# ChengZhang-98/lqer

Hardware: AMD Instinct MI355X
Metric: W4A8+rank-r Linear GEMM TFLOPS-equiv (higher is better)
Workload: dtype bf16; 1 GPU; LqerLinear 4096x4096 rank32 W4A8-MXINT16 M=2048 (BASELINE configs[1]); rank=32, formats=x MXINT8/16, W MXINT4/16, A_out,B_out as x, y fp16, weights=one Linear

## Files before the change

### lqer_amd/csrc/act16_fused.hip

```cpp
#include "common.h"

namespace lqer {
namespace a16f {

constexpr int ROWS = 8, WAVES = 8, SLAB = 512, PITCH = 1040;

__host__ inline size_t lds_bytes(int rp) { return (size_t)WAVES * ROWS * PITCH + (size_t)WAVES * ROWS * rp * sizeof(float); }

typedef __attribute__((ext_vector_type(8))) __bf16 bf16v8;

#ifdef LQER_CLOCKPROBE
__device__ unsigned long long* g_a16_stamp_buf = nullptr;
#define A16_STAMP(i) asm volatile("s_memtime %0\n\ts_waitcnt lgkmcnt(0)" : "=s"(cp[i])::"memory")
#else
#define A16_STAMP(i)
#endif

template <int DT, int RT>
__global__ __launch_bounds__(512) void k_act16_fused(const void* __restrict__ x, int64_t M, int64_t K, int64_t ld, QP qx, bf16_t* __restrict__ xq,
                                                      int64_t Kp, const bf16_t* __restrict__ a_frag, QP qa, int L_aout, bf16_t* __restrict__ xaq) {
  constexpr int RP = 16 * RT;
  constexpr int HB = RT == 8 ? 2 : (RT == 4 ? 4 : 8);
  constexpr int NPART = 16 / HB;
  extern __shared__ __attribute__((aligned(16))) unsigned char smem[];
  const int lane = threadIdx.x & 63;
  const int wave = __builtin_amdgcn_readfirstlane(threadIdx.x >> 6);
  unsigned char* const wb = smem + (size_t)wave * ROWS * PITCH;
  float* const red = (float*)(smem + (size_t)WAVES * ROWS * PITCH);
  const int64_t m0 = (int64_t)blockIdx.x * ROWS;
  const int nslab = (int)((Kp + SLAB - 1) / SLAB);
  const int g = lane >> 4;
  const unsigned char* const tok = wb + (lane & 7) * PITCH + 16 * g;
  const u32x4* const fr = (const u32x4*)a_frag + lane;
  f32x4 acc[RT];
#pragma unroll
  for (int t = 0; t < RT; ++t) acc[t] = (f32x4){0.f, 0.f, 0.f, 0.f};
#ifdef LQER_CLOCKPROBE
  unsigned long long cp[8] = {0, 0, 0, 0, 0, 0, 0, 0};
  A16_STAMP(0);
#endif

  for (int s = wave; s < nslab; s += WAVES) {
    const int64_t k0 = (int64_t)s * SLAB + 8 * lane;
    const bool in_img = k0 < Kp, in_x = k0 < K;
    u32x4 raw[ROWS];
#pragma unroll
    for (int r = 0; r < ROWS; ++r)
      raw[r] = (in_x && m0 + r < M) ? *(const u32x4*)((const bf16_t*)x + (m0 + r) * ld + k0) : (u32x4){0, 0, 0, 0};
    const int st0 = s * (SLAB / 32), nst = (int)(Kp / 32);
    u32x4 fa[HB][RT], fb[HB][RT];
    auto load_part = [&](u32x4 (&f)[HB][RT], int part) {
#pragma unroll
      for (int i = 0; i < HB; ++i)
#pragma unroll
        for (int t = 0; t < RT; ++t) {
          const int st = st0 + part * HB + i;
          f[i][t] = fr[((int64_t)(st < nst ? st : 0) * RT + t) * 64];
        }
    };
    if (s == wave) A16_STAMP(1);
#pragma unroll
    for (int r = 0; r < ROWS; ++r) {
      if (r == 1 && s == wave) A16_STAMP(2);
      if (r == 2) {
        asm volatile("" ::: "memory");
        load_part(fa, 0);
        asm volatile("" ::: "memory");
      }
      if (r == 5) {
        asm volatile("" ::: "memory");
        load_part(fb, 1);
        asm volatile("" ::: "memory");
      }
      float v[8];
      const uint32_t wd[4] = {raw[r][0], raw[r][1], raw[r][2], raw[r][3]};
#pragma unroll
      for (int j = 0; j < 4; ++j) {
        if constexpr (DT == LQER_F16) {
          typedef __attribute__((ext_vector_type(2))) _Float16 h2;
          const h2 h = __builtin_bit_cast(h2, wd[j]);
          v[2 * j] = (float)h[0], v[2 * j + 1] = (float)h[1];
        } else {
          v[2 * j] = __uint_as_float(wd[j] << 16), v[2 * j + 1] = __uint_as_float(wd[j] & 0xffff0000u);
        }
      }
      float amax = 0.f;
#pragma unroll
      for (int i = 0; i < 8; ++i) amax = fmaxf(amax, fabsf(v[i]));
      amax = fmaxf(amax, __shfl_xor(amax, 1, 64));
      uint32_t w[4] = {0, 0, 0, 0};
      if (amax > 0.f) {
        const int e = block_exponent_u(amax, qx);
        if (mxint16_fast_ok(e, qx)) {
          mxint16_bf16_fast<DT != LQER_F16, 8>(v, e, qx, w);
        } else {
#pragma unroll
          for (int i = 0; i < 4; ++i) {
            const uint32_t lo = exact_bf16_bits(ldexpf(mxint_mantissa(v[2 * i], e, qx), e - qx.mbits));
            const uint32_t hi = exact_bf16_bits(ldexpf(mxint_mantissa(v[2 * i + 1], e, qx), e - qx.mbits));
            w[i] = lo | (hi << 16);
          }
        }
      }
      const u32x4 wv = {w[0], w[1], w[2], w[3]};
      if (in_img) *(u32x4*)(xq + (m0 + r) * Kp + k0) = wv;
      *(u32x4*)(wb + r * PITCH + 16 * lane) = wv;
    }
    if (s == wave) A16_STAMP(3);
    __builtin_amdgcn_fence(__ATOMIC_RELEASE, "wavefront");
    __builtin_amdgcn_wave_barrier();
    __builtin_amdgcn_fence(__ATOMIC_ACQUIRE, "wavefront");
    auto half = [&](const u32x4 (&f)[HB][RT], int t0) {
      u32x4 tk[HB];
#pragma unroll
      for (int i = 0; i < HB; ++i) tk[i] = *(const u32x4*)(tok + 64 * (t0 + i));
#pragma unroll
      for (int i = 0; i < HB; ++i)
#pragma unroll
        for (int t = 0; t < RT; ++t)
          acc[t] = __builtin_amdgcn_mfma_f32_16x16x32_bf16(__builtin_bit_cast(bf16v8, tk[i]), __builtin_bit_cast(bf16v8, f[i][t]), acc[t], 0, 0, 0);
    };
#pragma unroll
    for (int pp = 0; pp < NPART; pp += 2) {
      half(fa, pp * HB);
      if (pp + 2 < NPART) load_part(fa, pp + 2);
      half(fb, (pp + 1) * HB);
      if (pp + 3 < NPART) load_part(fb, pp + 3);
    }
    __builtin_amdgcn_fence(__ATOMIC_RELEASE, "wavefront");
    __builtin_amdgcn_wave_barrier();
#ifdef LQER_CLOCKPROBE
    if (s == wave) {
      asm volatile("" ::"v"(acc[0]));
      A16_STAMP(4);
    }
#endif
  }
  if (g < 2) {
#pragma unroll
    for (int t = 0; t < RT; ++t)
#pragma unroll
      for (int j = 0; j < 4; ++j) red[(wave * ROWS + 4 * g + j) * RP + 16 * t + (lane & 15)] = acc[t][j];
  }
  __syncthreads();
#ifdef LQER_CLOCKPROBE
  A16_STAMP(5);
  if (g_a16_stamp_buf && lane == 0) {
    unsigned long long* o = g_a16_stamp_buf + ((size_t)blockIdx.x * WAVES + wave) * 8;
    for (int i = 1; i < 6; ++i) o[i] = cp[i] - cp[0];
    unsigned long long rt;
    asm volatile("s_memrealtime %0\n\ts_waitcnt lgkmcnt(0)" : "=s"(rt)::"memory");
    o[0] = cp[0], o[6] = rt;
  }
#endif
  const int tid = threadIdx.x;
  const bool live = tid < ROWS * RP / 4;
  const int r = tid / (RP / 4), c4 = tid - r * (RP / 4);
  float4 sum = make_float4(0.f, 0.f, 0.f, 0.f);
  if (live) {
#pragma unroll
    for (int w = 0; w < WAVES; ++w) {
      const float4 v = *(const float4*)(red + (w * ROWS + r) * RP + 4 * c4);
      sum.x += v.x, sum.y += v.y, sum.z += v.z, sum.w += v.w;
    }
  }
  if (tid >= 64 * ((ROWS * RP / 4 + 63) / 64)) return;
  float bmax = fmaxf(fmaxf(fabsf(sum.x), fabsf(sum.y)), fmaxf(fabsf(sum.z), fabsf(sum.w)));
  const int G = L_aout / 4;
  for (int d = 1; d < G; d <<= 1) bmax = fmaxf(bmax, __shfl_xor(bmax, d, 64));
  if (!live || m0 + r >= M) return;
  const bool anyb = bmax > 0.f;
  const int eb = anyb ? block_exponent(bmax, qa) : 0;
  const float v[4] = {sum.x, sum.y, sum.z, sum.w};
  uint32_t w2[2];
#pragma unroll
  for (int i = 0; i < 2; ++i) {
    const float m0v = anyb ? mxint_mantissa(v[2 * i], eb, qa) : 0.f;
    const float m1v = anyb ? mxint_mantissa(v[2 * i + 1], eb, qa) : 0.f;
    w2[i] = exact_bf16_bits(ldexpf(m0v, eb - qa.mbits)) | (exact_bf16_bits(ldexpf(m1v, eb - qa.mbits)) << 16);
  }
  *(uint2*)(xaq + ((m0 + r) * RP + 4 * c4)) = make_uint2(w2[0], w2[1]);
}

__global__ __launch_bounds__(256) void k_a_b16(const bf16_t* __restrict__ limb0, int64_t Kp, int rp, bf16_t* __restrict__ out) {
  const int RT = rp / 16;
  const int64_t n_img = (int64_t)rp * Kp / 8, total = 2 * n_img;
  for (int64_t idx = (int64_t)blockIdx.x * 256 + threadIdx.x; idx < total; idx += (int64_t)gridDim.x * 256) {
    if (idx < n_img) {
      ((u32x4*)out)[idx] = ((const u32x4*)limb0)[idx];
    } else {
      const int64_t f = idx - n_img;
      const int lane = (int)(f & 63);
      const int64_t blk = f >> 6;
      const int t = (int)(blk % RT);
      const int64_t s = blk / RT;
      ((u32x4*)out)[idx] = *(const u32x4*)(limb0 + (int64_t)(16 * t + (lane & 15)) * Kp + 32 * s + 8 * (lane >> 4));
    }
  }
}

}

#ifdef LQER_CLOCKPROBE
extern "C" int lqer_debug_set_a16_stamp_buffer(void* p) { return (int)hipMemcpyToSymbol(HIP_SYMBOL(a16f::g_a16_stamp_buf), &p, sizeof(p)); }
#endif

size_t a_b16_image_bytes(int64_t K, int64_t r) { return (size_t)2 * lqer_padded_r(r) * lqer_padded_k(K) * sizeof(bf16_t); }

int a_b16_prepare_dispatch(const void* a_t_limbs, int64_t K, int64_t r, void* out, hipStream_t st) {
  const int64_t rp = lqer_padded_r(r), Kp = lqer_padded_k(K);
  if (rp % 16 != 0 || Kp % 32 != 0) {
    set_error("a_b16_prepare: padded rank %d / padded K %d", (int)rp, (int)Kp);
    return LQER_E_UNSUPPORTED;
  }
  const int64_t total = 2 * rp * Kp / 8;
  a16f::k_a_b16<<<(unsigned)((total + 255) / 256 < 4096 ? (total + 255) / 256 : 4096), 256, 0, st>>>((const bf16_t*)a_t_limbs, Kp, (int)rp, (bf16_t*)out);
  return check_launch("a_b16_prepare");
}

int act16_fused_dispatch(const void* x, int dtype, int64_t M, int64_t K, int64_t ldx, const QP& qx, bf16_t* xq, const void* a_b16, int64_t r,
                         const QP& qa, bf16_t* xaq, int tuning, hipStream_t st) {
  if (tuning & LQER_TUNE_ACT16_SPLIT) return LQER_E_UNSUPPORTED;
  const int64_t rp = lqer_padded_r(r), Kp = lqer_padded_k(K);
  if (dtype == LQER_F32 || !a_b16 || !xaq || !xq || r <= 0 || M <= 0) return LQER_E_UNSUPPORTED;
  if (!(rp == 16 || rp == 32 || rp == 64)) return LQER_E_UNSUPPORTED;
  if (qx.kind != LQER_Q_MXINT || qx.block != 16 || qx.mbits > 8) return LQER_E_UNSUPPORTED;
  if (((uintptr_t)x % 16) != 0 || ((ldx * 2) % 16) != 0 || K % 16 != 0) return LQER_E_UNSUPPORTED;
  if (qa.kind != LQER_Q_MXINT || qa.mbits > 8) return LQER_E_UNSUPPORTED;
  const int L = (qa.block <= 0 || qa.block >= rp) ? (int)rp : qa.block;
  const int G = L / 4;
  if (rp % L != 0 || L % 4 != 0 || (G & (G - 1)) != 0 || G > 64) return LQER_E_UNSUPPORTED;
  if (!(tuning & LQER_TUNE_ACT16_FUSED) && (M > LQER_ACT8_FUSED_MAX_M || M < LQER_ACT8_FUSED_MIN_M)) return LQER_E_UNSUPPORTED;
  const bf16_t* const a_frag = (const bf16_t*)a_b16 + rp * Kp;
  const unsigned grid = (unsigned)((M + a16f::ROWS - 1) / a16f::ROWS);
  const int lds = (int)a16f::lds_bytes((int)rp);
  auto run = [&](auto dt) {
    constexpr int DT = decltype(dt)::value, LIMIT = 160 * 1024;
    const char* const what = "quantize_act_xa (fused block-16 route)";
    switch (rp / 16) {
      case 1: return launch_k<a16f::k_act16_fused<DT, 1>, LIMIT>(what, grid, 512, lds, st, x, M, K, ldx, qx, xq, Kp, a_frag, qa, L, xaq);
      case 2: return launch_k<a16f::k_act16_fused<DT, 2>, LIMIT>(what, grid, 512, lds, st, x, M, K, ldx, qx, xq, Kp, a_frag, qa, L, xaq);
      default: return launch_k<a16f::k_act16_fused<DT, 4>, LIMIT>(what, grid, 512, lds, st, x, M, K, ldx, qx, xq, Kp, a_frag, qa, L, xaq);
    }
  };
  return dtype == LQER_F16 ? run(std::integral_constant<int, LQER_F16>{}) : run(std::integral_constant<int, LQER_BF16>{});
}

}
```

Measured before the change: 1033 TFLOP/s-equiv.

## Software-pipeline act16 fused kernel: prefetch next slab and interleave quantize with MFMA

Restructures the fused block-16 activation quantize + X·A kernel so each lane handles 16-column pieces of two rows rather than one full row-slab. The x rows and A fragments for the next slab are prefetched at the end of the current one. Quantization pieces are interleaved with partial MFMA passes, with sched barriers fixing the order, so global loads overlap compute. A separate path for full slabs drops the per-element bounds checks. This adds register pressure from the prefetched buffers and uses clamped loads in place of zero-fill.

```diff
diff --git a/lqer_amd/csrc/act16_fused.hip b/lqer_amd/csrc/act16_fused.hip
--- a/lqer_amd/csrc/act16_fused.hip
+++ b/lqer_amd/csrc/act16_fused.hip
@@ -17,124 +17,169 @@
 #endif
 
 template <int DT, int RT>
-__global__ __launch_bounds__(512) void k_act16_fused(const void* __restrict__ x, int64_t M, int64_t K, int64_t ld, QP qx, bf16_t* __restrict__ xq,
-                                                      int64_t Kp, const bf16_t* __restrict__ a_frag, QP qa, int L_aout, bf16_t* __restrict__ xaq) {
+__global__ __launch_bounds__(512) void k_act16_fused(const void* __restrict__ x, int64_t M, int64_t ld, int64_t K, int64_t Kp,
+                                                      const bf16_t* __restrict__ a_frag, bf16_t* __restrict__ xq, bf16_t* __restrict__ xaq, QP qx, QP qa,
+                                                      int L_aout) {
   constexpr int RP = 16 * RT;
-  constexpr int HB = RT == 8 ? 2 : (RT == 4 ? 4 : 8);
-  constexpr int NPART = 16 / HB;
+  constexpr int QK = SLAB / 4, QS = QK / 32;
+  constexpr int HB = RT == 4 ? 2 : 4;
+  constexpr int NP = QS / HB;
   extern __shared__ __attribute__((aligned(16))) unsigned char smem[];
   const int lane = threadIdx.x & 63;
   const int wave = __builtin_amdgcn_readfirstlane(threadIdx.x >> 6);
+  const int64_t m0 = (int64_t)blockIdx.x * ROWS;
+#ifdef LQER_CLOCKPROBE
+  unsigned long long cp[8] = {0, 0, 0, 0, 0, 0, 0, 0};
+  A16_STAMP(0);
+#endif
+  const int rl = lane >> 4, cl = lane & 15;
+  const int nslab = (int)((Kp + SLAB - 1) / SLAB), nst = (int)(Kp / 32);
+  const bool row_ok[2] = {m0 + rl < M, m0 + 4 + rl < M};
+  const bf16_t* const xr[2] = {(const bf16_t*)x + (row_ok[0] ? m0 + rl : M - 1) * ld, (const bf16_t*)x + (row_ok[1] ? m0 + 4 + rl : M - 1) * ld};
+  const u32x4* const fr = (const u32x4*)a_frag + lane;
+  u32x4 raw[ROWS], fa[HB][RT], fb[HB][RT];
+  auto load_rows = [&](int s, auto j0, auto j1) {
+    asm volatile("" ::: "memory");
+#pragma unroll
+    for (int j = decltype(j0)::value; j < decltype(j1)::value; ++j) {
+      const int64_t k = (int64_t)s * SLAB + (j >> 1) * QK + 8 * cl;
+      raw[j] = *(const u32x4*)(xr[j & 1] + (k < K ? k : K - 8));
+    }
+    asm volatile("" ::: "memory");
+  };
+  auto load_part = [&](u32x4 (&f)[HB][RT], int s, int p) {
+    asm volatile("" ::: "memory");
+#pragma unroll
+    for (int i = 0; i < HB; ++i)
+#pragma unroll
+      for (int t = 0; t < RT; ++t) {
+        const int st = s * (SLAB / 32) + p * HB + i;
+        f[i][t] = fr[((int64_t)(st < nst ? st : 0) * RT + t) * 64];
+      }
+    asm volatile("" ::: "memory");
+  };
+  using I0 = std::integral_constant<int, 0>;
+  using I2 = std::integral_constant<int, 2>;
+  using I4 = std::integral_constant<int, 4>;
+  using I8 = std::integral_constant<int, 8>;
+  auto front = [&](int s) {
+    load_rows(s, I0{}, I2{});
+    load_part(fa, s, 0);
+    if constexpr (NP == 1) load_rows(s, I2{}, I4{});
+    load_part(fb, s, 1);
+    if constexpr (NP == 1) load_rows(s, I4{}, I8{});
+    else load_rows(s, I2{}, I8{});
+  };
+  if (wave < nslab) front(wave);
+  A16_STAMP(1);
   unsigned char* const wb = smem + (size_t)wave * ROWS * PITCH;
   float* const red = (float*)(smem + (size_t)WAVES * ROWS * PITCH);
-  const int64_t m0 = (int64_t)blockIdx.x * ROWS;
-  const int nslab = (int)((Kp + SLAB - 1) / SLAB);
   const int g = lane >> 4;
   const unsigned char* const tok = wb + (lane & 7) * PITCH + 16 * g;
-  const u32x4* const fr = (const u32x4*)a_frag + lane;
+  unsigned char* const wr[2] = {wb + rl * PITCH + 16 * cl, wb + (4 + rl) * PITCH + 16 * cl};
+  bf16_t* const xqr[2] = {xq + (m0 + rl) * Kp + 8 * cl, xq + (m0 + 4 + rl) * Kp + 8 * cl};
   f32x4 acc[RT];
 #pragma unroll
   for (int t = 0; t < RT; ++t) acc[t] = (f32x4){0.f, 0.f, 0.f, 0.f};
-#ifdef LQER_CLOCKPROBE
-  unsigned long long cp[8] = {0, 0, 0, 0, 0, 0, 0, 0};
-  A16_STAMP(0);
-#endif
-
-  for (int s = wave; s < nslab; s += WAVES) {
-    const int64_t k0 = (int64_t)s * SLAB + 8 * lane;
-    const bool in_img = k0 < Kp, in_x = k0 < K;
-    u32x4 raw[ROWS];
-#pragma unroll
-    for (int r = 0; r < ROWS; ++r)
-      raw[r] = (in_x && m0 + r < M) ? *(const u32x4*)((const bf16_t*)x + (m0 + r) * ld + k0) : (u32x4){0, 0, 0, 0};
-    const int st0 = s * (SLAB / 32), nst = (int)(Kp / 32);
-    u32x4 fa[HB][RT], fb[HB][RT];
-    auto load_part = [&](u32x4 (&f)[HB][RT], int part) {
-#pragma unroll
-      for (int i = 0; i < HB; ++i)
-#pragma unroll
-        for (int t = 0; t < RT; ++t) {
-          const int st = st0 + part * HB + i;
-          f[i][t] = fr[((int64_t)(st < nst ? st : 0) * RT + t) * 64];
+
+  auto piece = [&](int s, int j, auto full) {
+    constexpr bool FULL = decltype(full)::value;
+    const int64_t kq = (int64_t)s * SLAB + (j >> 1) * QK, k = kq + 8 * cl;
+    const bool live = row_ok[j & 1] && (FULL || k < K);
+    float v[8];
+    const uint32_t wd[4] = {live ? raw[j][0] : 0u, live ? raw[j][1] : 0u, live ? raw[j][2] : 0u, live ? raw[j][3] : 0u};
+#pragma unroll
+    for (int i = 0; i < 4; ++i) {
+      if constexpr (DT == LQER_F16) {
+        typedef __attribute__((ext_vector_type(2))) _Float16 h2;
+        const h2 h = __builtin_bit_cast(h2, wd[i]);
+        v[2 * i] = (float)h[0], v[2 * i + 1] = (float)h[1];
+      } else {
+        v[2 * i] = __uint_as_float(wd[i] << 16), v[2 * i + 1] = __uint_as_float(wd[i] & 0xffff0000u);
+      }
+    }
+    float amax = 0.f;
+#pragma unroll
+    for (int i = 0; i < 8; ++i) amax = fmaxf(amax, fabsf(v[i]));
+    amax = fmaxf(amax, __shfl_xor(amax, 1, 64));
+    uint32_t w[4] = {0, 0, 0, 0};
+    if (amax > 0.f) {
+      const int e = block_exponent_u(amax, qx);
+      if (mxint16_fast_ok(e, qx)) {
+        mxint16_bf16_fast<DT != LQER_F16, 8>(v, e, qx, w);
+      } else {
+#pragma unroll
+        for (int i = 0; i < 4; ++i) {
+          const uint32_t lo = exact_bf16_bits(ldexpf(mxint_mantissa(v[2 * i], e, qx), e - qx.mbits));
+          const uint32_t hi = exact_bf16_bits(ldexpf(mxint_mantissa(v[2 * i + 1], e, qx), e - qx.mbits));
+          w[i] = lo | (hi << 16);
         }
-    };
-    if (s == wave) A16_STAMP(1);
-#pragma unroll
-    for (int r = 0; r < ROWS; ++r) {
-      if (r == 1 && s == wave) A16_STAMP(2);
-      if (r == 2) {
-        asm volatile("" ::: "memory");
-        load_part(fa, 0);
-        asm volatile("" ::: "memory");
-      }
-      if (r == 5) {
-        asm volatile("" ::: "memory");
-        load_part(fb, 1);
-        asm volatile("" ::: "memory");
-      }
-      float v[8];
-      const uint32_t wd[4] = {raw[r][0], raw[r][1], raw[r][2], raw[r][3]};
-#pragma unroll
-      for (int j = 0; j < 4; ++j) {
-        if constexpr (DT == LQER_F16) {
-          typedef __attribute__((ext_vector_type(2))) _Float16 h2;
-          const h2 h = __builtin_bit_cast(h2, wd[j]);
-          v[2 * j] = (float)h[0], v[2 * j + 1] = (float)h[1];
-        } else {
-          v[2 * j] = __uint_as_float(wd[j] << 16), v[2 * j + 1] = __uint_as_float(wd[j] & 0xffff0000u);
-        }
-      }
-      float amax = 0.f;
-#pragma unroll
-      for (int i = 0; i < 8; ++i) amax = fmaxf(amax, fabsf(v[i]));
-      amax = fmaxf(amax, __shfl_xor(amax, 1, 64));
-      uint32_t w[4] = {0, 0, 0, 0};
-      if (amax > 0.f) {
-        const int e = block_exponent_u(amax, qx);
-        if (mxint16_fast_ok(e, qx)) {
-          mxint16_bf16_fast<DT != LQER_F16, 8>(v, e, qx, w);
-        } else {
-#pragma unroll
-          for (int i = 0; i < 4; ++i) {
-            const uint32_t lo = exact_bf16_bits(ldexpf(mxint_mantissa(v[2 * i], e, qx), e - qx.mbits));
-            const uint32_t hi = exact_bf16_bits(ldexpf(mxint_mantissa(v[2 * i + 1], e, qx), e - qx.mbits));
-            w[i] = lo | (hi << 16);
-          }
-        }
-      }
-      const u32x4 wv = {w[0], w[1], w[2], w[3]};
-      if (in_img) *(u32x4*)(xq + (m0 + r) * Kp + k0) = wv;
-      *(u32x4*)(wb + r * PITCH + 16 * lane) = wv;
-    }
-    if (s == wave) A16_STAMP(3);
+      }
+    }
+    const u32x4 wv = {w[0], w[1], w[2], w[3]};
+    if (FULL || k < Kp) *(u32x4*)(xqr[j & 1] + kq) = wv;
+    *(u32x4*)(wr[j & 1] + 256 * (j >> 1)) = wv;
+    __builtin_amdgcn_sched_barrier(0);
+  };
+  auto mult = [&](const u32x4 (&f)[HB][RT], int p) {
     __builtin_amdgcn_fence(__ATOMIC_RELEASE, "wavefront");
     __builtin_amdgcn_wave_barrier();
     __builtin_amdgcn_fence(__ATOMIC_ACQUIRE, "wavefront");
-    auto half = [&](const u32x4 (&f)[HB][RT], int t0) {
-      u32x4 tk[HB];
-#pragma unroll
-      for (int i = 0; i < HB; ++i) tk[i] = *(const u32x4*)(tok + 64 * (t0 + i));
-#pragma unroll
-      for (int i = 0; i < HB; ++i)
-#pragma unroll
-        for (int t = 0; t < RT; ++t)
-          acc[t] = __builtin_amdgcn_mfma_f32_16x16x32_bf16(__builtin_bit_cast(bf16v8, tk[i]), __builtin_bit_cast(bf16v8, f[i][t]), acc[t], 0, 0, 0);
-    };
-#pragma unroll
-    for (int pp = 0; pp < NPART; pp += 2) {
-      half(fa, pp * HB);
-      if (pp + 2 < NPART) load_part(fa, pp + 2);
-      half(fb, (pp + 1) * HB);
-      if (pp + 3 < NPART) load_part(fb, pp + 3);
-    }
+    __builtin_amdgcn_sched_barrier(0);
+    u32x4 tk[HB];
+#pragma unroll
+    for (int i = 0; i < HB; ++i) tk[i] = *(const u32x4*)(tok + 64 * (HB * p + i));
+#pragma unroll
+    for (int i = 0; i < HB; ++i)
+#pragma unroll
+      for (int t = 0; t < RT; ++t)
+        acc[t] = __builtin_amdgcn_mfma_f32_16x16x32_bf16(__builtin_bit_cast(bf16v8, tk[i]), __builtin_bit_cast(bf16v8, f[i][t]), acc[t], 0, 0, 0);
     __builtin_amdgcn_fence(__ATOMIC_RELEASE, "wavefront");
     __builtin_amdgcn_wave_barrier();
+    __builtin_amdgcn_sched_barrier(0);
+  };
+  auto slab = [&](int s, auto full) {
+    [[maybe_unused]] const bool first = s == wave;
+    piece(s, 0, full), piece(s, 1, full);
+    if (first) A16_STAMP(2);
+    if constexpr (NP == 1) {
+      mult(fa, 0);
+      load_part(fa, s, 2);
+      piece(s, 2, full), piece(s, 3, full);
+      mult(fb, 1);
+      load_part(fb, s, 3);
+      piece(s, 4, full), piece(s, 5, full);
+      mult(fa, 2);
+      piece(s, 6, full), piece(s, 7, full);
+      if (first) A16_STAMP(3);
+      mult(fb, 3);
+    } else {
+      mult(fa, 0);
+      load_part(fa, s, 2);
+      mult(fb, 1);
+      load_part(fb, s, 3);
+#pragma unroll
+      for (int j = 2; j < 8; ++j) piece(s, j, full);
+      if (first) A16_STAMP(3);
+#pragma unroll
+      for (int p = 2; p < 4 * NP; p += 2) {
+        mult(fa, p);
+        if (p + 2 < 4 * NP) load_part(fa, s, p + 2);
+        mult(fb, p + 1);
+        if (p + 3 < 4 * NP) load_part(fb, s, p + 3);
+      }
+    }
+  };
+  for (int s = wave; s < nslab; s += WAVES) {
+    if ((int64_t)(s + 1) * SLAB <= K) slab(s, std::true_type{});
+    else slab(s, std::false_type{});
 #ifdef LQER_CLOCKPROBE
     if (s == wave) {
       asm volatile("" ::"v"(acc[0]));
       A16_STAMP(4);
     }
 #endif
+    if (s + WAVES < nslab) front(s + WAVES);
   }
   if (g < 2) {
 #pragma unroll
@@ -238,9 +283,9 @@
     constexpr int DT = decltype(dt)::value, LIMIT = 160 * 1024;
     const char* const what = "quantize_act_xa (fused block-16 route)";
     switch (rp / 16) {
-      case 1: return launch_k<a16f::k_act16_fused<DT, 1>, LIMIT>(what, grid, 512, lds, st, x, M, K, ldx, qx, xq, Kp, a_frag, qa, L, xaq);
-      case 2: return launch_k<a16f::k_act16_fused<DT, 2>, LIMIT>(what, grid, 512, lds, st, x, M, K, ldx, qx, xq, Kp, a_frag, qa, L, xaq);
-      default: return launch_k<a16f::k_act16_fused<DT, 4>, LIMIT>(what, grid, 512, lds, st, x, M, K, ldx, qx, xq, Kp, a_frag, qa, L, xaq);
+      case 1: return launch_k<a16f::k_act16_fused<DT, 1>, LIMIT>(what, grid, 512, lds, st, x, M, ldx, K, Kp, a_frag, xq, xaq, qx, qa, L);
+      case 2: return launch_k<a16f::k_act16_fused<DT, 2>, LIMIT>(what, grid, 512, lds, st, x, M, ldx, K, Kp, a_frag, xq, xaq, qx, qa, L);
+      default: return launch_k<a16f::k_act16_fused<DT, 4>, LIMIT>(what, grid, 512, lds, st, x, M, ldx, K, Kp, a_frag, xq, xaq, qx, qa, L);
     }
   };
   return dtype == LQER_F16 ? run(std::integral_constant<int, LQER_F16>{}) : run(std::integral_constant<int, LQER_BF16>{});
```

Result: faster. 1052 TFLOP/s-equiv, median of 6 (+1.9%).
